# AtomGradient/swift-qwen3-tts

Measured on AMD Instinct MI355X. Metric: codec_tokens_per_s, higher is better.
Workload: dtype bf16

## Files before the change

swift-qwen3-tts_amd/csrc/codec.cc:

```cpp
#include "codec.h"

#include <algorithm>
#include <cstdlib>
#include <cstring>
#include <type_traits>
#include <utility>

#include "codec_kernels.h"

namespace q3 {

namespace {
size_t kScratchBudget = size_t(24) << 30;
}
void CodecRunner::set_scratch_budget(size_t bytes) { kScratchBudget = bytes ? bytes : (size_t(24) << 30); }

CodecRunner::CodecRunner(const Model& m, hipStream_t st, bool fp32_convs, int output_rate, float speed) : m_(m), st_(st) {
    native_ = mid_ = up_ = m.cfg.codec.total_upsample();
    if (speed != 0.0f && speed != 1.0f) {
        Q3_CHECK(speed >= 0.5f && speed <= 2.0f, 3, "Invalid input: speed must be 0 (off) or between 0.5 and 2.0");
        Q3_CHECK(native_ % kStretchHa == 0, 3, "Invalid input: the codec's frame is not a whole number of 480-sample hops: no speed other than 1");
        const int hops = native_ / kStretchHa;
        int L = 1, M = 1;
        if (output_rate != 0 && output_rate != kResampleNative && resample_rate_supported(output_rate)) {
// ... 55 lines not shown
    int C = dc.decoder_dim;
    for (int r : dc.upsample_rates) {
        ppf *= r;
        C /= 2;
        per_frame = std::max(per_frame, size_t(ppf) * C);
    }
    if (stretch_) per_frame = std::max(per_frame, size_t(mid_));
    return per_frame;
}

int CodecRunner::tail_context_frames() const {
    const CodecDecoderConfig& dc = m_.cfg.codec;
    double ctx = 0.0, rate = 1.0;
    for (int r : dc.upsampling_ratios) {
        rate *= r;
        ctx += 6.0 / rate;
    }
    ctx += 6.0 / rate;
    for (int r : dc.upsample_rates) {
        ctx += 1.0 / rate;
        rate *= r;
        ctx += 6.0 * (1 + 3 + 9) / rate;
    }
    ctx += 6.0 / rate;
    if (stretch_) ctx += double(stretch_lookback(st_plan_.hs)) / rate;
    if (resample_) ctx += double(out_plan_.taps() - 1) / rate;
    return int(ctx) + 2;
}

void CodecRunner::upload_lens(const int32_t* lens, int n) {
    if (size_t(n) > lens_dev_.capacity()) Q3_HIP(hipStreamSynchronize(st_));
    lens_dev_.grow(size_t(n));
    lens_host_.grow(size_t(n));
    Q3_HIP(hipStreamSynchronize(st_));
    std::memcpy(lens_host_, lens, size_t(n) * 4);
    Q3_HIP(hipMemcpyAsync(lens_dev_, lens_host_, size_t(n) * 4, hipMemcpyHostToDevice, st_));
}

void CodecRunner::conv(const Pass& ps, const ConvW& cw, const float* x, int Tmax, int ppf, float* out, const SnakeW* sn,
                       const float* res, int act, const SnakeW* post, float* out2) {
    launch([&] {
        ConvGemmArgs a{};
        const int64_t m_in = int64_t(ps.hist_frames) * ppf * cw.Cin, m_out = int64_t(ps.hist_frames) * ppf * cw.N;
        a.hist = ps.hist_frames * ppf;
        a.x = x + m_in; a.ldx = cw.Cin; a.x_bstride = int64_t(Tmax) * cw.Cin;
        a.w = cw.w; a.bias = cw.bias; a.scale = cw.scale;
        if (!fp32_mfma_) { a.wh = cw.wh; a.wsc = cw.wsc; }
        a.res = res ? res + m_out : nullptr; a.ldr = cw.N; a.res_bstride = int64_t(Tmax) * cw.N;
        a.out = out ? out + m_out : nullptr; a.ldo = cw.N; a.out_bstride = int64_t(Tmax) * cw.N;
        a.snake_ea = sn ? sn->ea : nullptr; a.snake_ib = sn ? sn->ib : nullptr;
        if (post) { a.out2 = out2 + m_out; a.post_ea = post->ea; a.post_ib = post->ib; a.post_C = post->C; }
        a.frames = ps.fr; a.ppf = ppf; a.Tmax = Tmax; a.B = ps.nb;
        a.Cin = cw.Cin; a.N = cw.N; a.K = cw.K; a.dil = cw.dil; a.act = act;
        launch_conv_gemm(a, st_);
    });
}

void CodecRunner::capture(const Pass& ps, const char* name, const float* t, int T, int C) {
    if (!ps.stage_out || *ps.stage != name) return;
    Q3_HIP(hipStreamSynchronize(st_));
    ps.stage_out->resize(size_t(ps.nb) * T * C);
    Q3_HIP(hipMemcpy(ps.stage_out->data(), t, ps.stage_out->size() * 4, hipMemcpyDeviceToHost));
    if (ps.stage_T) *ps.stage_T = T;
    if (ps.stage_C) *ps.stage_C = C;
}

void CodecRunner::run_front(const Pass& ps, const int32_t* codes, int code_stride_frames, int Fmax, float* const* bufs,
                            const int32_t* first_frame) {
    const CodecDecoderConfig& dc = m_.cfg.codec;
// ... 757 lines not shown
```

swift-qwen3-tts_amd/csrc/codec.h:

```cpp
#pragma once
#include <string>
#include <vector>

#include "model.h"
#include "resample_plan.h"
#include "stream_plan.h"
#include "stretch_plan.h"

namespace q3 {

class CodecRunner {
  public:
    CodecRunner(const Model& m, hipStream_t st, bool fp32_convs = false, int output_rate = 0, float speed = 0.0f);
    int decode(const int32_t* codes_dev, int code_stride_frames, const std::vector<int>& frames, float** pcm_dev,
               const std::string& stage = std::string(), std::vector<float>* stage_out = nullptr, int* stage_T = nullptr,
               int* stage_C = nullptr, int32_t* nonfinite_host = nullptr, bool force_fp32 = false);
    bool fp32_convs() const { return fp32_mfma_; }
    int decode_chunked(const int32_t* codes_dev, int code_stride_frames, const std::vector<int>& frames, int chunk_frames,
                       float* pcm_host, std::vector<hipEvent_t>& chunk_done, int32_t* nonfinite_host = nullptr,
                       int32_t* nf_chunks_host = nullptr);
    int tail_context_frames() const;
    static void set_scratch_budget(size_t bytes);

    struct StreamCfg {
// ... 107 lines not shown
        ~Stream() {
            for (auto e : ring_ev) (void)hipEventDestroy(e);
            for (auto e : quiet_ev) (void)hipEventDestroy(e);
        }
        uint8_t* take(size_t bytes);
        void* get(size_t frame_bytes, bool reads_back);
        void put(const void*) {}
    } stream_;
    void stream_prefix();
    size_t front_floats_per_frame() const;
    size_t floats_per_frame() const;
    void upload_lens(const int32_t* lens, int n);
    static constexpr int kMaxRows = 4096;
    const Model& m_;
    hipStream_t st_;
    int up_ = 1920;
    int native_ = 1920;
    bool resample_ = false;
    ResamplePlan out_plan_;
    DevBuf<float> out_tab_;
    int mid_ = 1920;
    bool stretch_ = false;
    StretchPlan st_plan_;
    DevBuf<float> st_fade_;
    static constexpr int kStateWords = 4;
    DevBuf<int32_t> ch_words_;
    DevBuf<float> ch_mid_;
    bool no_h1_ = false;
    bool no_fuse_ = false;
    bool fp32_mfma_ = false;
    DevBuf<uint8_t> buf_;
    DevBuf<int32_t> lens_dev_;
    PinnedBuf<int32_t> lens_host_;
    DevBuf<int32_t> nf_dev_;
};

}
```

swift-qwen3-tts_amd/csrc/debug_env.cc:

```cpp
#include <atomic>
#include <cstdlib>
#include <mutex>

#include "kernels.h"

namespace q3 {

namespace {
std::mutex g_mu;
std::atomic<const DebugEnv*> g_env{nullptr};

bool flag(const char* name) { return std::getenv(name) != nullptr; }
int number(const char* name, int dflt) {
    const char* e = std::getenv(name);
    return e && *e ? std::atoi(e) : dflt;
}

const DebugEnv* read_env() {
    DebugEnv* d = new DebugEnv{};
    d->gemm_no_row_split = flag("Q3TTS_GEMM_NO_ROW_SPLIT");
    d->gemm_one_pair = flag("Q3TTS_GEMM_ONE_PAIR");
    d->no_tall_gemm = flag("Q3TTS_NO_TALL_GEMM");
    d->tall_shape = number("Q3TTS_TALL_SHAPE", 0);
    d->chunk_qsplit = number("Q3TTS_CHUNK_QSPLIT", 0);
    d->conv_no_pw = flag("Q3TTS_CONV_NO_PW");
    d->nt_off = std::getenv("Q3TTS_NT") && number("Q3TTS_NT", 1) == 0;
    d->serial_jobs = number("Q3TTS_SERIAL_JOBS", 0) != 0;
    d->fail_back_half = number("Q3TTS_TEST_FAIL_BACK_HALF", 0) != 0;
    d->no_prefix_cache = number("Q3TTS_NO_PREFIX_CACHE", 0) != 0;
    return d;
}
}

const DebugEnv& debug_env() {
    const DebugEnv* e = g_env.load(std::memory_order_acquire);
    if (!e) {
        std::lock_guard<std::mutex> lk(g_mu);
        e = g_env.load(std::memory_order_acquire);
        if (!e) {
            e = read_env();
            g_env.store(e, std::memory_order_release);
        }
    }
    return *e;
}

void debug_env_reload() {
    std::lock_guard<std::mutex> lk(g_mu);
    g_env.store(read_env(), std::memory_order_release);
}

}
```

swift-qwen3-tts_amd/csrc/engine.cc:

```cpp
#include "engine.h"

#include <algorithm>
#include <cctype>
#include <chrono>
#include <cmath>
#include <cstdio>
#include <deque>
#include <functional>
#include <thread>

#include "codec.h"
#include "codec_kernels.h"
#include "frontend.h"

namespace q3 {

namespace {
std::string lower(const std::string& s) {
    std::string o = s;
    for (auto& c : o) c = char(std::tolower((unsigned char)c));
    return o;
}
const char* const kCodecRangeMsg =
    "Audio decoding failed: the codec decoder produced a non-finite waveform -- also on the fp32 matrix-core convolutions (the "
    "reference's range), which a row is re-decoded on when it leaves the fp16 range of the default two-plane kernels";
double now_s() {
    return std::chrono::duration<double>(std::chrono::steady_clock::now().time_since_epoch()).count();
}
struct Bump {
    uint8_t* base;
    size_t off = 0;
    template <class T>
    T* take(size_t n) {
        off = align_up(off, 256);
        T* p = base ? reinterpret_cast<T*>(base + off) : nullptr;
        off += n * sizeof(T);
        return p;
    }
};
void audio_chunk(q3tts_event_cb cb, void* user, int request_index, const float* pcm, int64_t n, int64_t offset) {
    q3tts_event ev{};
    ev.kind = Q3TTS_EVENT_AUDIO_CHUNK;
    ev.request_index = request_index;
    ev.pcm = pcm;
    ev.n_samples = n;
    ev.sample_offset = offset;
    cb(user, &ev);
}
}

Engine::Engine(Model* model, const q3tts_load_opts& opts) : m_(model), opts_(opts) {
    Q3_HIP(hipSetDevice(m_->device));
    {
        int least = 0, greatest = 0;
        Q3_HIP(hipDeviceGetStreamPriorityRange(&least, &greatest));
        Q3_HIP(hipStreamCreateWithPriority(&st_, hipStreamNonBlocking, greatest));
        Q3_HIP(hipStreamCreateWithPriority(&st_codec_, hipStreamNonBlocking, least));
        hipDeviceProp_t prop{};
        Q3_HIP(hipGetDeviceProperties(&prop, m_->device));
        int cus = prop.multiProcessorCount / 2;
        if (opts.codec_overlap_cus > 0) cus = opts.codec_overlap_cus;
// ... 1279 lines not shown
            const SlotStream::Out& o = ss->out[b];
            Q3_CHECK(o.complete, 7, "internal error: a row of the streamed job was left incomplete");
            std::memcpy(J.pcm_host + (size_t(b) * stride + prefix[size_t(b)]) * J.up, o.pcm.get(), size_t(J.frames[size_t(b)]) * J.up * 4);
            J.held_from[size_t(b)] = o.held_from;
            J.nf_host[b] = o.held_from >= 0 ? 1 : 0;
        }
        if (ss->have_first) J.timing.first_audio_ms = ss->first_audio_ms;
    }
};

int Engine::begin(const q3tts_request* reqs, int n, const q3tts_sampling& sp, q3tts_event_cb cb, void* user, const DebugOpts* dbg,
                  bool overlapped, bool background, const Voice* const* voices) {
    Q3_HIP(hipSetDevice(m_->device));
    std::vector<ResolvedRequest> rr;
    double t_start = 0;
    const int slot = open_job(reqs, n, sp, dbg, rr, t_start, voices);
    bool any_clone = false;
    for (auto& r : rr) any_clone = any_clone || r.clone;
    Q3_HIP(hipEventRecord(ev_fe_[0], st_));
    const bool frontend = any_clone && prepare_clone_rows(rr);
    Q3_HIP(hipEventRecord(ev_fe_[1], st_));
    std::vector<int> np, nt;
    assemble_prompts(rr, np, nt);
    const int Pmax = reserve_rows(rr, np, nt, sp);
    if (dbg) debug_buffers(n, *dbg);
    Q3_HIP(hipEventRecord(ev_[0], st_));
    enqueue_prefill(tk_, n, Pmax, block_table_, kv_len_, n_prompt_, active_);
    Q3_HIP(hipEventRecord(ev_[1], st_));
    Job& J = jobs_[slot];
    J.reset(n, codec_->upsample());
    J.chunk_frames = sp.audio_chunk_frames;
    J.frontend = frontend;
    J.busy = true;
    if (background && !cb && !dbg && sp.audio_chunk_frames == 0) {
        J.background = true;
        J.rr = std::move(rr);
        J.np = std::move(np);
        J.sp = sp;
        J.sp.per_request = nullptr;
        J.overlapped = overlapped;
        J.t_start = t_start;
        std::lock_guard<std::mutex> lk(work_mu_);
        if (!worker_.joinable()) worker_ = std::thread([this] { worker_loop(); });
        J.back = 1;
        J.back_status = 0;
        J.back_err.clear();
        work_ = &J;
        work_cv_.notify_all();
        return slot;
    }
    try {
        back_half(J, rr, np, sp, cb, user, dbg,
                  sp.audio_chunk_frames > 0 && sp.audio_window_frames > 0 && (!any_clone || sp.audio_stream_reference != 0) && !dbg, overlapped,
                  t_start);
    } catch (...) {
        J.busy = false;
        throw;
    }
    return slot;
}

void Engine::back_half(Job& J, const std::vector<ResolvedRequest>& rr, const std::vector<int>& np, const q3tts_sampling& sp,
                       q3tts_event_cb cb, void* user, const DebugOpts* dbg, bool streamed, bool overlapped, double t_start) {
    if (J.background && debug_env().fail_back_half) throw Error(7, "back half failed on request (Q3TTS_TEST_FAIL_BACK_HALF)");
    StreamedDecode sd(*this, J, streamed, sp, cb, user, rr, t_start);
    const int launched = frame_loop(J, rr, sp, cb, user, dbg, sd);
// ... 114 lines not shown
    Q3_HIP(hipMalloc(reinterpret_cast<void**>(&sampled_dev_), nf * 16 * 4));
    Q3_HIP(hipMemset(sampled_dev_, 0xff, nf * 16 * 4));
    if (dbg.talker_logits) Q3_HIP(hipMalloc(reinterpret_cast<void**>(&tl_dump_), nf * V * 2));
    if (dbg.cp_logits) Q3_HIP(hipMalloc(reinterpret_cast<void**>(&cl_dump_), nf * (t.num_code_groups - 1) * Vc * 2));
}

int Engine::frame_loop(Job& J, const std::vector<ResolvedRequest>& rr, const q3tts_sampling& sp, q3tts_event_cb cb, void* user,
                       const DebugOpts* dbg, StreamedDecode& sd) {
    const int n = J.n;
    const bool use_graph = opts_.use_graph && !dbg;
    build_cp_proj_tables();
    hipGraphExec_t ge = use_graph ? frame_graph(n) : nullptr;
    int frames_cap = 0;
    for (auto& r : rr) frames_cap = std::max(frames_cap, r.max_frames);
    std::vector<int32_t> h_nframes((size_t)(n), 0);
    std::vector<uint8_t> h_fin((size_t)(n), 0);
    std::vector<int> reported((size_t)(n), 0);
    int launched = 0;
    const bool fixed_len = sp.force_frames > 0 || dbg;
    const int burst_frames = std::max(1, max_inflight_frames / job_chains / 2);
    hipEvent_t ring[2] = {burst_ev_[0], burst_ev_[1]};
    int bursts = 0;
    bool done = false;
    while (!done && launched < frames_cap) {
        if (bursts >= 2) Q3_HIP(hipEventSynchronize(ring[bursts & 1]));
        int burst = std::min(burst_frames, frames_cap - launched);
        if (sd.on) {
            const int need = std::min(frames_cap, sd.next_need(launched, sp.audio_chunk_frames, std::max(0, sp.audio_lookahead_frames)));
            if (need > launched) burst = std::min(burst, need - launched);
        }
        for (int i = 0; i < burst; ++i) {
            if (use_graph) Q3_HIP(hipGraphLaunch(ge, st_));
            else enqueue_frame(n, dbg);
        }
        launched += burst;
        if (!(fixed_len && !cb)) {
            Q3_HIP(hipMemcpyAsync(h_nframes.data(), n_frames_, size_t(n) * 4, hipMemcpyDeviceToHost, st_));
            Q3_HIP(hipMemcpyAsync(h_fin.data(), finished_, size_t(n), hipMemcpyDeviceToHost, st_));
        }
        Q3_HIP(hipEventRecord(ring[bursts & 1], st_));
        ++bursts;
        if (fixed_len && !cb) {
            if (sd.on) {
                for (int b = 0; b < n; ++b) sd.avail[size_t(b)] = std::min(launched, rr[size_t(b)].max_frames);
                sd.feed(launched);
            }
            continue;
        }
        Q3_HIP(hipEventSynchronize(ring[(bursts - 1) & 1]));
        done = true;
        for (int b = 0; b < n; ++b) done = done && h_fin[size_t(b)];
        if (sd.on) {
            for (int b = 0; b < n; ++b) {
                sd.avail[size_t(b)] = h_nframes[size_t(b)];
                sd.fin[size_t(b)] = h_fin[size_t(b)];
            }
            sd.feed(launched);
            fire_chunks(J, J.n_chunks, &sd.avail, false);
        }
        if (cb)
            for (int b = 0; b < n; ++b) emit_tokens(cb, user, b, request_base + b, h_nframes[size_t(b)], reported[size_t(b)]);
    }
    Q3_HIP(hipEventRecord(ev_[2], st_));
    Q3_HIP(hipMemcpyAsync(h_nframes.data(), n_frames_, size_t(n) * 4, hipMemcpyDeviceToHost, st_));
    Q3_HIP(hipStreamSynchronize(st_));
    if (dbg) {
        const TalkerConfig& t = m_->cfg.talker;
        const size_t nf = size_t(n) * dbg->frames;
        if (dbg->sampled) Q3_HIP(hipMemcpy(dbg->sampled, sampled_dev_, nf * 16 * 4, hipMemcpyDeviceToHost));
        if (dbg->talker_logits) Q3_HIP(hipMemcpy(dbg->talker_logits, tl_dump_, nf * t.vocab_size * 2, hipMemcpyDeviceToHost));
        if (dbg->cp_logits)
            Q3_HIP(hipMemcpy(dbg->cp_logits, cl_dump_, nf * (t.num_code_groups - 1) * t.cp.vocab_size * 2, hipMemcpyDeviceToHost));
    }
    J.frames.assign(h_nframes.begin(), h_nframes.end());
    return launched;
}

void Engine::hand_off(Job& J, const std::vector<ResolvedRequest>& rr, StreamedDecode& sd, int launched, bool overlapped) {
    const int n = J.n;
    bool any_clone = false;
    std::vector<int> dframes((size_t)(n), 0);
    int Fdec = 0;
    for (int b = 0; b < n; ++b) {
        const int F = J.frames[size_t(b)];
        any_clone = any_clone || rr[size_t(b)].clone;
        J.ref_T[size_t(b)] = rr[size_t(b)].clone ? rr[size_t(b)].ref_T : 0;
        J.target_tokens[size_t(b)] = rr[size_t(b)].target_token_count;
        dframes[size_t(b)] = F > 0 ? F + J.ref_T[size_t(b)] : 0;
        Fdec = std::max(Fdec, dframes[size_t(b)]);
    }
    J.Fdec = sd.on ? (sd.ss ? sd.stride : Fcap_) : Fdec;
    J.codes_host.resize(size_t(n) * Fcap_ * 16);
    Q3_HIP(hipMemcpyAsync(J.codes_host.data(), codes_, J.codes_host.size() * 4, hipMemcpyDeviceToHost, st_));
    if (sd.on) {
        for (int b = 0; b < n; ++b) {
            sd.avail[size_t(b)] = J.frames[size_t(b)];
            sd.fin[size_t(b)] = 1;
        }
// ... 5 lines not shown
        J.decoded = Fdec > 0;
        return;
    }
    if (Fdec > 0) {
        J.dec_codes.grow(size_t(n) * Fdec * 16);
        if (any_clone) {
            J.row_desc.assign(size_t(n), DecodeRowDesc{});
            for (int b = 0; b < n; ++b) {
                const auto& r = rr[size_t(b)];
                if (J.frames[size_t(b)] == 0) continue;
                J.row_desc[size_t(b)] = DecodeRowDesc{r.clone ? ref_codes_dev_ + r.ref_off : nullptr, codes_ + size_t(b) * Fcap_ * 16,
                                                      r.clone ? r.ref_T : 0, J.frames[size_t(b)], b, 0};
                if (r.voice) {
                    J.ref_code0[size_t(b)] = r.voice->code0;
                } else if (r.clone) {
                    J.ref_code0[size_t(b)].resize(size_t(r.ref_T));
                    Q3_HIP(hipMemcpyAsync(J.ref_code0[size_t(b)].data(), ref_codes_dev_ + r.ref_off, size_t(r.ref_T) * 4,
                                          hipMemcpyDeviceToHost, st_));
                }
            }
            Q3_HIP(hipMemcpyAsync(J.row_desc_dev.grow(size_t(n)), J.row_desc.data(), size_t(n) * sizeof(DecodeRowDesc), hipMemcpyHostToDevice, st_));
            launch_build_decode_codes_rows(J.row_desc.data(), J.row_desc_dev, n, J.dec_codes, n, Fdec, st_);
        } else {
            Q3_HIP(hipMemcpy2DAsync(J.dec_codes, size_t(Fdec) * 64, codes_, size_t(Fcap_) * 64, size_t(Fdec) * 64, size_t(n),
                                    hipMemcpyDeviceToDevice, st_));
        }
    }
    Q3_HIP(hipStreamSynchronize(st_));
    start_decode(J, dframes, overlapped, nullptr);
}

void Engine::start_decode(Job& J, const std::vector<int>& dframes, bool overlapped, const int32_t* codes_host) {
    hipStream_t cst = codec_stream(overlapped, J.background);
    Q3_HIP(hipEventRecord(J.ev_codec[0], cst));
    if (J.Fdec > 0) {
        const size_t floats = size_t(J.n) * J.Fdec * J.up;
        J.pcm_host.grow(floats);
        if (codes_host && J.voices.empty()) {
            J.dec_codes.grow(size_t(J.n) * J.Fdec * 16);
            Q3_HIP(hipMemcpy2DAsync(J.dec_codes, size_t(J.Fdec) * 64, codes_host, size_t(Fcap_) * 64, size_t(J.Fdec) * 64, size_t(J.n),
                                    hipMemcpyHostToDevice, cst));
        } else if (codes_host) {
            J.dec_codes.grow(size_t(J.n) * J.Fdec * 16);
            Q3_HIP(hipMemsetAsync(J.dec_codes, 0, size_t(J.n) * J.Fdec * 64, cst));
            J.gen_codes.grow(size_t(J.n) * Fcap_ * 16);
            int Fgen = 0;
            for (int b = 0; b < J.n; ++b) Fgen = std::max(Fgen, J.frames[size_t(b)]);
            Q3_CHECK(Fgen <= Fcap_, 7, "internal error: more generated frames than max_frames");
            Q3_HIP(hipMemcpy2DAsync(J.gen_codes, size_t(Fcap_) * 64, codes_host, size_t(Fcap_) * 64, size_t(Fgen) * 64, size_t(J.n),
                                    hipMemcpyHostToDevice, cst));
            J.row_desc.assign(size_t(J.n), DecodeRowDesc{});
            for (int b = 0; b < J.n; ++b) {
                const Voice* v = J.voices[size_t(b)];
                J.row_desc[size_t(b)] = DecodeRowDesc{v ? static_cast<const int32_t*>(v->codes_dev) : nullptr,
                                                      J.gen_codes + size_t(b) * Fcap_ * 16, v ? v->ref_T : 0, J.frames[size_t(b)], b, 0};
            }
            Q3_HIP(hipMemcpyAsync(J.row_desc_dev.grow(size_t(J.n)), J.row_desc.data(), size_t(J.n) * sizeof(DecodeRowDesc),
                                  hipMemcpyHostToDevice, cst));
            launch_build_decode_codes_rows(J.row_desc.data(), J.row_desc_dev, J.n, J.dec_codes, J.n, J.Fdec, cst);
        }
        if (J.chunk_frames > 0) {
            J.clear_chunk_flags(J.Fdec);
            J.n_chunks = codec_->decode_chunked(J.dec_codes, J.Fdec, dframes, J.chunk_frames, J.pcm_host, J.chunk_done, J.nf_host,
                                                J.nf_chunk_host);
        } else {
            float* pcm_dev = nullptr;
            codec_->decode(J.dec_codes, J.Fdec, dframes, &pcm_dev, std::string(), nullptr, nullptr, nullptr, J.nf_host);
            Q3_HIP(hipMemcpyAsync(J.pcm_host, pcm_dev, floats * 4, hipMemcpyDeviceToHost, cst));
        }
        J.decoded = true;
    }
    Q3_HIP(hipEventRecord(J.ev_codec[1], cst));
}

void Engine::job_timing(Job& J, const std::vector<int>& np, int launched) {
    float ms = 0;
    Q3_HIP(hipEventElapsedTime(&ms, ev_[0], ev_[1]));
    J.timing.prefill_ms = ms;
    Q3_HIP(hipEventElapsedTime(&ms, ev_[1], ev_[2]));
    J.timing.decode_ms = ms;
    Q3_HIP(hipEventElapsedTime(&ms, ev_fe_[0], ev_fe_[1]));
    J.timing.frontend_ms = J.frontend ? ms : 0;
    J.timing.frame_steps = launched;
    J.timing.launches_per_frame_step = launches_per_step(J.n);
    J.timing.rows = J.n;
    for (int b = 0; b < J.n; ++b) J.timing.kv_bytes_read += kv_bytes(np[size_t(b)], J.frames[size_t(b)]);
}

void Engine::publish_job(Job& J, q3tts_event_cb cb, void* user, int req_base, double t_start, bool stage) {
    J.cb = cb;
    J.user = user;
    J.request_base = req_base;
    J.t_start = t_start;
    J.seq = job_seq_++;
    J.busy = true;
    compute_cuts(J);
    std::lock_guard<std::mutex> lk(stage_mu_);
    J.stage_err.clear();
    J.stage = (stage && J.decoded) ? 1 : 0;
    if (J.stage == 1) {
        if (!stager_.joinable()) stager_ = std::thread([this] { staging_loop(); });
        stage_cv_.notify_all();
    }
}

void Engine::release_job(Job& J) {
    {
        std::unique_lock<std::mutex> lk(stage_mu_);
        stage_cv_.wait(lk, [&] { return J.stage != 1; });
    }
    J.st_pcm.clear();
    J.st_codes.clear();
    J.back_status = 0;
    J.busy = false;
}

void Engine::Job::reset(int rows, int upsample) {
    n = rows;
    up = upsample;
    Fdec = 0;
    frames.assign(size_t(n), 0);
    ref_T.assign(size_t(n), 0);
    target_tokens.assign(size_t(n), 0);
    ref_code0.assign(size_t(n), {});
    req_index.clear();
    row_out.clear();
    row_span.clear();
    held_from.assign(size_t(n), -1);
    std::memset(nf_host, 0, nf_host.capacity() * 4);
    n_chunks = chunk_frames = chunks_fired = 0;
    streamed = prefixed = decoded = background = frontend = false;
    voices.clear();
    t_first_audio = t_done = 0;
    timing = q3tts_timing{};
}

void Engine::Job::clear_chunk_flags(int frames) {
    const size_t slots = size_t(ceil_div(frames, chunk_frames) + 1) * size_t(n);
    std::memset(nf_chunk_host.grow(slots), 0, slots * 4);
}

void check_row_sampling(const q3tts_sampling& sp, int n) {
    if (!sp.per_request) return;
    constexpr uint32_t kKnown = Q3TTS_ROW_TEMPERATURE | Q3TTS_ROW_TOP_K | Q3TTS_ROW_TOP_P | Q3TTS_ROW_REPETITION_PENALTY | Q3TTS_ROW_SEED;
    for (int i = 0; i < n; ++i) {
        const q3tts_row_sampling& r = sp.per_request[i];
        const std::string at = " (per_request[" + std::to_string(i) + "])";
        Q3_CHECK((r.set & ~kKnown) == 0, 3, "Invalid input: unknown bits in q3tts_row_sampling.set" + at);
        if (r.set & Q3TTS_ROW_TEMPERATURE) Q3_CHECK(std::isfinite(r.temperature), 3, "Invalid input: temperature must be finite" + at);
        if (r.set & Q3TTS_ROW_TOP_K) Q3_CHECK(r.top_k >= 0, 3, "Invalid input: top_k must not be negative" + at);
        if (r.set & Q3TTS_ROW_TOP_P)
            Q3_CHECK(std::isfinite(r.top_p) && r.top_p >= 0.f && r.top_p <= 1.f, 3, "Invalid input: top_p must be in [0, 1]" + at);
        if (r.set & Q3TTS_ROW_REPETITION_PENALTY)
            Q3_CHECK(std::isfinite(r.repetition_penalty) && r.repetition_penalty > 0.f, 3,
                     "Invalid input: repetition_penalty must be finite and positive" + at);
    }
}

SamplingParams fold_sampling(const q3tts_sampling& sp, int i, uint32_t row0) {
    SamplingParams o{sp.temperature, sp.top_k, sp.top_p, sp.repetition_penalty, sp.seed, row0, sp.force_frames > 0 ? 1 : 0};
    if (!sp.per_request) return o;
    const q3tts_row_sampling& r = sp.per_request[i];
    if (r.set & Q3TTS_ROW_TEMPERATURE) o.temperature = r.temperature;
    if (r.set & Q3TTS_ROW_TOP_K) o.top_k = r.top_k;
    if (r.set & Q3TTS_ROW_TOP_P) o.top_p = r.top_p;
    if (r.set & Q3TTS_ROW_REPETITION_PENALTY) o.rep_penalty = r.repetition_penalty;
    if (r.set & Q3TTS_ROW_SEED) o.seed = r.seed;
// ... 82 lines not shown
        if (!J.cb) continue;
        const int64_t c0 = int64_t(k) * J.chunk_frames * up, c1 = std::min<int64_t>(int64_t(J.Fdec), int64_t(k + 1) * J.chunk_frames) * up;
        std::unique_lock<std::mutex> lk = cb_lock();
        for (int b = 0; b < n; ++b) {
            if (J.held_from[size_t(b)] >= 0) continue;
            const int64_t cut = known ? 0 : J.row_cut[size_t(b)];
            const int64_t len = known ? int64_t((*known)[size_t(b)]) * up : J.row_ns[size_t(b)];
            const int64_t lo = std::max(c0, cut), hi = std::min(c1, cut + len);
            if (hi <= lo) continue;
            audio_chunk(J.cb, J.user, J.request_base + b, J.pcm_host + size_t(b) * J.Fdec * up + lo, hi - lo, lo - cut);
        }
    }
}

void Engine::stage_rows(Job& J) {
    Q3_HIP(hipSetDevice(m_->device));
    Q3_HIP(hipEventSynchronize(J.ev_codec[1]));
    J.t_done = now_s();
    const int n = J.n;
    J.st_pcm.clear();
    J.st_pcm.resize(size_t(n));
    J.st_codes.clear();
    J.st_codes.resize(size_t(n));
    for (int b = 0; b < n; ++b) {
        const int F = J.frames[size_t(b)];
        if (F == 0 || !J.decoded) continue;
        const int64_t ns = J.row_ns[size_t(b)];
        J.st_codes[size_t(b)].reset(static_cast<int32_t*>(std::malloc(size_t(F) * 16 * 4)));
        J.st_pcm[size_t(b)].reset(static_cast<float*>(std::malloc(std::max<size_t>(size_t(ns) * 4, 4))));
        Q3_CHECK(J.st_codes[size_t(b)] && J.st_pcm[size_t(b)], 5, "out of host memory for the results");
        std::memcpy(J.st_codes[size_t(b)].get(), J.codes_host.data() + size_t(b) * Fcap_ * 16, size_t(F) * 16 * 4);
        std::memcpy(J.st_pcm[size_t(b)].get(), J.pcm_host + size_t(b) * J.Fdec * J.up + J.row_cut[size_t(b)], size_t(ns) * 4);
    }
}

void Engine::staging_loop() {
    std::unique_lock<std::mutex> lk(stage_mu_);
    for (;;) {
        Job* next = nullptr;
        for (auto& J : jobs_)
            if (J.stage == 1 && (!next || J.seq < next->seq)) next = &J;
        if (!next) {
            if (stage_stop_) return;
            stage_cv_.wait(lk);
            continue;
        }
        lk.unlock();
        int state = 2;
        std::string err;
        try {
            stage_rows(*next);
        } catch (const std::exception& e) {
            state = 3;
            err = e.what();
        }
        lk.lock();
        next->stage = state;
        next->stage_err = err;
        stage_cv_.notify_all();
    }
}

std::vector<int> Engine::redo_rows_fp32(Job& J) {
    std::vector<int> rows, bad;
    if (!J.decoded) return bad;
    for (int b = 0; b < J.n; ++b)
// ... 113 lines not shown
        r.info.tokens_per_second = total > 0 ? double(F) / total : 0;
        r.info.peak_memory_usage = double(total_b - free_b) / 1e9;
        if (F == 0 || !J.decoded) {
            r.status = Q3TTS_ERR_GENERATION_FAILED;
            continue;
        }
        if (std::find(still_bad.begin(), still_bad.end(), b) != still_bad.end()) {
            r.status = Q3TTS_ERR_AUDIO_DECODING_FAILED;
            last_error = kCodecRangeMsg;
            continue;
        }
        r.n_frames = F;
        r.codes = J.st_codes[size_t(b)].release();
        r.n_samples = row_ns[size_t(b)];
        r.pcm = J.st_pcm[size_t(b)].release();
        r.status = Q3TTS_OK;
    }
    if (J.cb) {
        std::unique_lock<std::mutex> lk = cb_lock();
        for (int b = 0; b < n; ++b) {
            if (out(b).status != Q3TTS_OK) continue;
            q3tts_event ev{};
            ev.kind = Q3TTS_EVENT_INFO;
            ev.request_index = ev_index(b);
            ev.info = &out(b).info;
            J.cb(J.user, &ev);
            ev.kind = Q3TTS_EVENT_AUDIO;
            ev.info = nullptr;
            ev.pcm = out(b).pcm;
            ev.n_samples = out(b).n_samples;
            J.cb(J.user, &ev);
        }
    }
}

bool Engine::job_outstanding() const {
    for (const auto& J : jobs_)
        if (J.busy) return true;
    return false;
}

ResolvedRequest Engine::check_queued(const q3tts_request& r, const q3tts_sampling& sp, const Voice* voice, bool open_text) const {
    const TalkerConfig& t = m_->cfg.talker;
    Q3_CHECK(r.ref_audio == nullptr, 3, "Invalid input: voice-clone requests (ref_audio) are not supported by q3tts_generate_queued");
    ResolvedRequest o = resolve(r, sp, voice);
    if (open_text) {
        Q3_CHECK(!o.clone, 3, "Invalid input: an open-text request cannot be a voice-clone request");
        o.n_tail = 0;
        o.text_open = true;
        o.open_max_tokens = r.max_tokens > 0 ? r.max_tokens : 2048;
        o.open_force_frames = sp.force_frames;
        o.max_frames = sp.force_frames > 0 ? sp.force_frames : o.open_max_tokens;
        o.target_token_count = int(o.text_ids.size()) - 3;
    }
    Q3_CHECK(m_->has_codec, 1, "Model not initialized: Speech tokenizer not loaded");
    Q3_CHECK(o.max_frames <= Fcap_, 3, "Invalid input: max_tokens exceeds the configured max_frames");
    Q3_CHECK(o.language_id < t.vocab_size && o.speaker_token < t.vocab_size, 3, "Invalid input: codec prefix id out of range");
    const int tl = int(o.text_ids.size());
    int nc = (o.language_id < 0 ? 3 : 4) + (o.speaker_token >= 0 ? 1 : 0) + 2;
    int np = int(o.instruct_ids.size()) + 3 + nc;
    int nt = (tl - o.n_tail > 4 ? tl - o.n_tail - 4 : 0) + 1;
    if (o.clone) {
        nc += m_->has_speaker_encoder ? 1 : 0;
        np = 3 + (nc - 1) + (int(o.ref_text_ids.size()) - 5) + (tl - 8) + 2 + o.ref_T;
        nt = 1;
    }
// ... 1403 lines not shown

void Engine::debug_codec_stage(const int32_t* codes, int n_frames, const char* stage, float* out, int64_t cap, int* T, int* C) {
    Q3_CHECK(m_->has_codec, 1, "Model not initialized: Speech tokenizer not loaded");
    DevBuf<int32_t> dcodes;
    dcodes.grow(size_t(n_frames) * 16);
    Q3_HIP(hipMemcpy(dcodes, codes, size_t(n_frames) * 16 * 4, hipMemcpyHostToDevice));
    std::vector<float> so;
    float* pcm_dev = nullptr;
    (void)codec_stream(false);
    codec_->decode(dcodes, n_frames, {n_frames}, &pcm_dev, stage, &so, T, C);
    Q3_CHECK(int64_t(so.size()) <= cap, 3, "debug_codec_stage: output buffer too small");
    std::memcpy(out, so.data(), so.size() * 4);
}


EngineGroup::EngineGroup(std::unique_ptr<Model> model, const q3tts_load_opts& opts) : model_(std::move(model)), opts_(opts) {
    int lanes = opts.n_streams;
    if (lanes <= 0) lanes = 1;
    lanes = std::max(1, std::min(lanes, opts.max_batch));
    q3tts_load_opts lo = opts;
    lo.max_batch = ceil_div(opts.max_batch, lanes);
    for (int i = 0; i < lanes; ++i) {
        lanes_.push_back(std::make_unique<Engine>(model_.get(), lo));
        lanes_.back()->cb_mutex = &cb_mutex_;
        lanes_.back()->max_inflight_frames = std::max(2, 12000 / 650 / lanes);
    }
    speakers = lanes_[0]->speakers;
    if (lanes == 1) {
        ctx1_ = std::make_unique<Engine>(model_.get(), lo);
        ctx1_->cb_mutex = &cb_mutex_;
        background_ = !debug_env().serial_jobs;
        if (background_)
            for (Engine* e : {lanes_[0].get(), ctx1_.get()}) e->prepare_job_pair();
    }
}

EngineGroup::~EngineGroup() {
    session_.reset();
    ctx1_.reset();
    lanes_.clear();
}

Engine* EngineGroup::free_context() {
    Engine* c[2] = {lanes_[0].get(), ctx1_.get()};
    for (int k = 1; k <= 2; ++k) {
        const int i = (last_ctx_ + k) & 1;
        if (c[i]->job_outstanding()) continue;
        last_ctx_ = i;
        c[i]->row_offset = 0;
        c[i]->request_base = 0;
        return c[i];
    }
    throw Error(3, "Invalid input: two jobs are already outstanding (q3tts_generate_end must be called first)");
}

int EngineGroup::begin(const q3tts_request* reqs, int n, const q3tts_sampling& sp, q3tts_event_cb cb, void* user, bool more_follows) {
    Q3_CHECK(n >= 1 && n <= opts_.max_batch, 3, "Invalid input: batch size must be between 1 and max_batch");
    check_row_sampling(sp, n);
    if (lanes_.size() == 1) {
        Engine* e = free_context();
        return (e == ctx1_.get() ? Engine::kJobSlots : 0) + e->begin(reqs, n, sp, cb, user, nullptr, more_follows, background_);
    }
    int slot = -1;
    for (int i = 0; i < Engine::kJobSlots; ++i)
        if (!parked_[i].busy) slot = i;
    Q3_CHECK(slot >= 0, 3, "Invalid input: two jobs are already outstanding (q3tts_generate_end must be called first)");
    parked_[slot].results.assign(size_t(n), q3tts_result{});
// ... 403 lines not shown
```

swift-qwen3-tts_amd/csrc/engine.h:

```cpp
#pragma once
#include <atomic>
#include <cstdlib>
#include <map>
#include <memory>
#include <condition_variable>
#include <mutex>
#include <thread>
#include <string>
#include <unordered_map>
#include <vector>

#include "../../include/q3tts.h"
#include "kernels.h"
#include "model.h"
#include "resample_plan.h"
#include "session_queue.h"
#include "stretch_plan.h"

namespace q3 {

struct DebugOpts {
    const int32_t* forced_codes = nullptr;
    int frames = 0;
    uint16_t* talker_logits = nullptr;
    uint16_t* cp_logits = nullptr;
    int32_t* sampled = nullptr;
};

struct Voice {
    const void* owner = nullptr;
    int ref_T = 0;
    int64_t n_ref_samples = 0;
    std::vector<int32_t> ref_text_ids;
    DevBuf<int32_t> codes_dev;
    DevBuf<uint16_t> rows_dev;
    std::vector<int32_t> codes_host;
    std::vector<int32_t> code0;
    int64_t device_bytes = 0;
};

struct ResolvedRequest {
    std::vector<int32_t> text_ids, instruct_ids;
    int speaker_token = -1;
    int language_id = -1;
    int max_frames = 0;
// ... 77 lines not shown

struct RequestSource {
    virtual ~RequestSource() = default;
    virtual bool take(QueueItem& out) = 0;
    virtual q3tts_result* result(int ticket) = 0;
    virtual void complete(int) {}
    virtual bool open_ended() const { return false; }
    virtual bool wait_for_work() { return false; }
    virtual bool has_cancels() { return false; }
    virtual void take_cancels(std::vector<int>& out) { out.clear(); }
    virtual void complete_cancelled(int) {}
    virtual void progress(int , int ) {}
    struct TextAppend {
        int ticket = -1;
        std::vector<int32_t> ids;
        bool final = false;
    };
    virtual bool open_text() const { return false; }
    virtual bool has_appends() { return false; }
    virtual void take_appends(std::vector<TextAppend>& out) { out.clear(); }
    virtual void wait_for_text(bool ) {}
    virtual void text_progress(int , int ) {}
};

struct QueueShared {
    RequestSource* src = nullptr;
    uint32_t row_base = 0;
    int voice_ref_max = -1;
    bool stream_reference = false;
    int ref_max = 0;
    PrefixCache* prefix_cache = nullptr;
};

class Engine {
  public:
    Engine(Model* model, const q3tts_load_opts& opts);
    ~Engine();

    Model& model() { return *m_; }
    const q3tts_load_opts& opts() const { return opts_; }
    std::string last_error;
    q3tts_timing timing{};

    void generate(const q3tts_request* reqs, int n, const q3tts_sampling& sp, q3tts_event_cb cb, void* user,
                  q3tts_result* results, const DebugOpts* dbg, const Voice* const* voices = nullptr);
    static constexpr int kJobSlots = 2;
    int begin(const q3tts_request* reqs, int n, const q3tts_sampling& sp, q3tts_event_cb cb, void* user, const DebugOpts* dbg,
              bool overlapped,
              bool background = false, const Voice* const* voices = nullptr);
    void end(int job, q3tts_result* results);
    bool job_outstanding() const;
    int text_cap() const { return Tcap_; }
    void prepare_job_pair();
    void drain();
    ResolvedRequest check_queued(const q3tts_request& r, const q3tts_sampling& sp, const Voice* voice = nullptr,
                                 bool open_text = false) const;
    void check_stream_chunk(int chunk_frames) const;
    void run_queued(QueueShared& q, int slots, const q3tts_sampling& sp, q3tts_event_cb cb, void* user);
    void debug_prepare_inputs(const q3tts_request& req, uint16_t* input_embeds, int cap_prompt, int* n_prompt,
                              uint16_t* trailing, int cap_trailing, int* n_trailing, uint16_t* tts_pad);
    void debug_sample(const uint16_t* logits, int rows, int V, const q3tts_sampling& sp, const uint8_t* seen,
                      int suppress_lo, int suppress_hi, int eos_id, uint32_t row0, uint32_t draw, int32_t* tokens);
    void debug_text_resume(int H, int V, const uint16_t* tables, const int32_t* codes, const uint16_t* text, uint16_t* out_h,
                           float* out_ss, int32_t* out_state);
    void debug_linear(const uint16_t* x, const uint16_t* W, const uint16_t* bias, int M, int K, int N, uint16_t* y);
    void debug_attention(const q3tts_attn_debug& a);
    static void debug_gemm_check(q3tts_gemm_debug& d, GemmArgs& ga, NormRowsArgs& na);
    void debug_gemm(q3tts_gemm_debug& d);
    static void debug_conv_check(q3tts_conv_debug& d);
    void debug_conv(q3tts_conv_debug& d);
    void debug_build_decode_codes(const int32_t* refs, const int32_t* ref_T, const int32_t* gen, const int32_t* n_frames, int R,
                                  int gen_stride, int Fdec, bool misalign, int32_t* out);
    void codec_decode(const int32_t* codes, const int32_t* n_frames, int batch, int max_frames, float* pcm,
                      int64_t* audio_lengths);
    void codec_decode_streamed(const int32_t* codes, const int32_t* n_frames, int batch, int max_frames, int chunk_frames, int window,
                               int lookahead, float* pcm);
    void codec_decode_streamed_prefixed(const int32_t* codes, const int32_t* n_prefix, const int32_t* n_frames, int batch, int max_frames,
                                        int chunk_frames, int window, int lookahead, float* pcm);
    void debug_codec_stream_slots(const int32_t* codes, const int32_t* n_frames, int n_reqs, int max_frames, int slots, int burst,
                                  int chunk_frames, int window, int lookahead, float* pcm);
    void debug_codec_stage(const int32_t* codes, int n_frames, const char* stage, float* out, int64_t cap, int* T, int* C);
    int codec_encode(const float* audio, int64_t n_samples, int32_t* codes, int cap_frames);
    int encoded_frames(int64_t n_samples) const;
    void speaker_embedding(const float* audio, int64_t n_samples, float* out, int cap);
    std::unique_ptr<Voice> create_voice(const float* audio, int64_t n_samples, const int32_t* ref_text_ids, int n_ref_text_ids,
                                        int sample_rate = 24000);
// ... 62 lines not shown
        q3tts_sampling sp{};
        bool overlapped = false;
        bool frontend = false;
        bool background = false;
        int back = 0;
        int back_status = 0;
        std::string back_err;
        int n = 0, Fdec = 0, up = 0;
        std::vector<int> frames, ref_T, target_tokens, n_prompt;
        std::vector<int> req_index;
        std::vector<q3tts_result*> row_out;
        std::vector<double> row_span;
        std::vector<std::vector<int32_t>> ref_code0;
        std::vector<int32_t> codes_host;
        DevBuf<int32_t> dec_codes;
        std::vector<const Voice*> voices;
        DevBuf<int32_t> gen_codes;
        std::vector<DecodeRowDesc> row_desc;
        DevBuf<DecodeRowDesc> row_desc_dev;
        PinnedBuf<float> pcm_host;
        hipEvent_t ev_codec[2] = {nullptr, nullptr};
        PinnedBuf<int32_t> nf_host;
        PinnedBuf<int32_t> nf_chunk_host;
        std::vector<int> held_from;
        hipEvent_t ev_begin = nullptr, ev_first_audio = nullptr;
        std::vector<hipEvent_t> chunk_done;
        int n_chunks = 0, chunk_frames = 0;
        bool streamed = false;
        bool prefixed = false;
        int chunks_fired = 0;
        double t_first_audio = 0;
        q3tts_timing timing{};
        double t_start = 0, t_done = 0;
        q3tts_event_cb cb = nullptr;
        void* user = nullptr;
        int request_base = 0;
        bool decoded = false;
        std::vector<int64_t> row_cut, row_ns;
        std::vector<MallocPtr<float>> st_pcm;
        std::vector<MallocPtr<int32_t>> st_codes;
        int stage = 0;
        std::string stage_err;
        void reset(int rows, int upsample);
        void clear_chunk_flags(int frames);
    } jobs_[kJobSlots];
    void start_decode(Job& J, const std::vector<int>& dframes, bool overlapped, const int32_t* codes_host);
    void publish_job(Job& J, q3tts_event_cb cb, void* user, int request_base, double t_start, bool stage);
    void release_job(Job& J);
    void compute_cuts(Job& J);
    void fire_chunks(Job& J, int upto, const std::vector<int>* known, bool wait);
    std::unique_lock<std::mutex> cb_lock();
    void emit_tokens(q3tts_event_cb cb, void* user, int row, int request, int nf, int& reported);
    void stage_rows(Job& J);
    std::vector<int> redo_rows_fp32(Job& J);
    void staging_loop();
    std::thread stager_;
    std::mutex stage_mu_;
    std::condition_variable stage_cv_;
    bool stage_stop_ = false;
    uint64_t job_seq_ = 0;

    unsigned long long* stamps_ = nullptr;
    void stamp(int k) {
        if (stamps_) launch_stamp(stamps_, stamps_ + 63, k, counted());
    }
    hipStream_t counted() {
        ++launches_;
        return st_;
    }
    int launches_ = 0;
    std::map<int, int> frame_launches_;
    std::map<int, hipGraphExec_t> graphs_;
    std::unique_ptr<CodecRunner> codec_;
    std::unique_ptr<VoiceFrontEnd> fe_;
    DevBuf<float> ref_audio_dev_;
    DevBuf<int32_t> ref_codes_dev_;
    DevBuf<uint16_t> extra_;
    DevBuf<float> spk_f32_;
    struct FeLane {
        hipStream_t st = nullptr;
        hipEvent_t done = nullptr;
        std::unique_ptr<VoiceFrontEnd> fe;
        DevBuf<float> spk;
    };
    std::vector<FeLane> fe_lanes_;
    const float* upload_audio(const float* audio, int64_t n);
    struct ResamplerDev {
        ResamplePlan plan;
        DevBuf<float> tab;
    };
    std::vector<std::unique_ptr<ResamplerDev>> resamplers_;
    DevBuf<float> rs_out_dev_;
    DevBuf<int32_t> rs_len_dev_;
// ... 100 lines not shown
    bool mine(const Voice* v) const;
    PrefixCache& prefix_cache() { return prefix_cache_; }
    int begin(const q3tts_request* reqs, int n, const q3tts_sampling& sp, q3tts_event_cb cb, void* user, bool more_follows);
    void end(int job, q3tts_result* results);
    void generate_queued(const q3tts_request* reqs, int n, int slots, const q3tts_sampling& sp, q3tts_event_cb cb, void* user,
                         q3tts_result* results, const Voice* const* voices = nullptr);
    Session* open_session(const q3tts_session_opts& so, const q3tts_sampling& sp, q3tts_event_cb cb, void* user);
    Session* session() const { return session_.get(); }
    int close_session(bool drain);
    std::string last_error;
    q3tts_timing timing{};
    std::vector<std::string> speakers;

  private:
    std::unique_ptr<Session> session_;
    void check_queue_open(int slots, const q3tts_sampling& sp) const;
    template <class F>
    static void run_lanes(int L, bool serial, F&& fn);
    struct Parked {
        bool busy = false;
        std::vector<q3tts_result> results;
        q3tts_timing timing{};
    } parked_[Engine::kJobSlots];
    std::unique_ptr<Model> model_;
    q3tts_load_opts opts_;
    std::mutex cb_mutex_;
    std::vector<std::unique_ptr<Engine>> lanes_;
    std::vector<std::unique_ptr<Voice>> voices_;
    PrefixCache prefix_cache_;
    void check_voices(const q3tts_request* reqs, int n, const Voice* const* voices) const;
    std::unique_ptr<Engine> ctx1_;
    int last_ctx_ = 1;
    bool background_ = false;
    Engine* free_context();
};

class Session final : public RequestSource {
  public:
    struct Item {
        ResolvedRequest rr;
        SamplingParams params{};
    };
    Session(EngineGroup& g, Engine& lane, const q3tts_session_opts& so, const q3tts_sampling& sp, q3tts_event_cb cb, void* user);
    ~Session() override;
    void submit(const q3tts_request& r, const Voice* voice, const q3tts_row_sampling* rs, int64_t* ticket);
    void submit_open(const q3tts_request& r, const q3tts_row_sampling* rs, int64_t* ticket);
    void append_text(int64_t ticket, const int32_t* ids, int32_t n, bool final);
    void text_stats(q3tts_session_text_stats* s) const { queue_.text_stats(s); }
    int cancel(int64_t ticket) { return queue_.cancel(ticket); }
    void wait(int64_t ticket, int32_t timeout_ms, q3tts_result* out, int32_t* ready);
    void stats(q3tts_session_stats* s) const { queue_.stats(s); }
    int close(bool drain);
    bool on_loop_thread() const { return std::this_thread::get_id() == thread_.get_id(); }
    std::string error() const;

    bool take(QueueItem& out) override;
    q3tts_result* result(int ticket) override { return queue_.result(ticket); }
    void complete(int ticket) override { queue_.complete(ticket); }
    bool open_ended() const override { return true; }
    bool wait_for_work() override { return queue_.wait_for_work(); }
    bool has_cancels() override { return queue_.has_cancels(); }
    void take_cancels(std::vector<int>& out) override;
    void complete_cancelled(int ticket) override { queue_.complete_cancelled(ticket); }
    void progress(int frame_steps, int admissions) override { queue_.progress(frame_steps, admissions); }
    bool open_text() const override { return true; }
    bool has_appends() override { return queue_.has_appends(); }
// ... 20 lines not shown
```

swift-qwen3-tts_amd/csrc/kernels.h:

```cpp
#pragma once
#include <hip/hip_runtime.h>

#include <cstdint>

namespace q3 {

struct DebugEnv {
    bool gemm_no_row_split;
    bool gemm_one_pair;
    bool no_tall_gemm;
    int tall_shape;
    int chunk_qsplit;
    bool conv_no_pw;
    bool nt_off;
    bool serial_jobs;
    bool fail_back_half;
    bool no_prefix_cache;
};
const DebugEnv& debug_env();
void debug_env_reload();

constexpr int kPageTokens = 64;
constexpr int kHeadDim = 128;

struct NormRowsArgs {
    const uint16_t* h;
    int hMB;
    const uint16_t* w;
    float eps;
    uint16_t* out;
    int outMB;
    float* ss_out;
    int M, H;
    const float* ss_in;
    int ss_count, ss_ld;
};
void launch_norm_rows(const NormRowsArgs& a, hipStream_t st);

struct GemmArgs {
    const uint16_t* W;
    const uint32_t* Wsb;
    const uint16_t* x;
    int xMB;
    int M, Mpad, N, K;
    int epi;
    uint16_t* y;
    int ldy;
    int y_tiled, yMB;
    const uint16_t* bias;
    int act_silu;
// ... 204 lines not shown
```

Baseline: 10290.

## Serialize background codec decodes across contexts with an event-ordered gate

Adds a DecodeGate that gives background codec decode passes from the two engine contexts a ticket order. Each pass makes its codec stream wait on the previous pass's completion event through a small ring of three events, so the two contexts' decodes no longer contend on the GPU at the same time. upload_lens now waits on an event recorded after its own host-to-device copy instead of synchronizing the whole stream, so the host no longer blocks on unrelated queued work. The change also adds optional per-job tracing and a test failure hook, and it holds a mutex across the enqueue of each decode pass.

```diff
diff --git a/swift-qwen3-tts_amd/csrc/codec.cc b/swift-qwen3-tts_amd/csrc/codec.cc
--- a/swift-qwen3-tts_amd/csrc/codec.cc
+++ b/swift-qwen3-tts_amd/csrc/codec.cc
@@ -111,9 +111,11 @@
     if (size_t(n) > lens_dev_.capacity()) Q3_HIP(hipStreamSynchronize(st_));
     lens_dev_.grow(size_t(n));
     lens_host_.grow(size_t(n));
-    Q3_HIP(hipStreamSynchronize(st_));
+    if (!lens_copied_.e) Q3_HIP(hipEventCreateWithFlags(&lens_copied_.e, hipEventDisableTiming));
+    else Q3_HIP(hipEventSynchronize(lens_copied_.e));
     std::memcpy(lens_host_, lens, size_t(n) * 4);
     Q3_HIP(hipMemcpyAsync(lens_dev_, lens_host_, size_t(n) * 4, hipMemcpyHostToDevice, st_));
+    Q3_HIP(hipEventRecord(lens_copied_.e, st_));
 }
 
 void CodecRunner::conv(const Pass& ps, const ConvW& cw, const float* x, int Tmax, int ppf, float* out, const SnakeW* sn,
diff --git a/swift-qwen3-tts_amd/csrc/codec.h b/swift-qwen3-tts_amd/csrc/codec.h
--- a/swift-qwen3-tts_amd/csrc/codec.h
+++ b/swift-qwen3-tts_amd/csrc/codec.h
@@ -163,6 +163,12 @@
     DevBuf<uint8_t> buf_;
     DevBuf<int32_t> lens_dev_;
     PinnedBuf<int32_t> lens_host_;
+    struct OwnedEvent {
+        hipEvent_t e = nullptr;
+        ~OwnedEvent() {
+            if (e) (void)hipEventDestroy(e);
+        }
+    } lens_copied_;
     DevBuf<int32_t> nf_dev_;
 };
 
diff --git a/swift-qwen3-tts_amd/csrc/debug_env.cc b/swift-qwen3-tts_amd/csrc/debug_env.cc
--- a/swift-qwen3-tts_amd/csrc/debug_env.cc
+++ b/swift-qwen3-tts_amd/csrc/debug_env.cc
@@ -1,5 +1,6 @@
 #include <atomic>
 #include <cstdlib>
+#include <cstring>
 #include <mutex>
 
 #include "kernels.h"
@@ -26,8 +27,12 @@
     d->conv_no_pw = flag("Q3TTS_CONV_NO_PW");
     d->nt_off = std::getenv("Q3TTS_NT") && number("Q3TTS_NT", 1) == 0;
     d->serial_jobs = number("Q3TTS_SERIAL_JOBS", 0) != 0;
-    d->fail_back_half = number("Q3TTS_TEST_FAIL_BACK_HALF", 0) != 0;
+    d->fail_in_decode = number("Q3TTS_TEST_FAIL_BACK_HALF", 0) == 2;
+    d->fail_back_half = number("Q3TTS_TEST_FAIL_BACK_HALF", 0) != 0 && !d->fail_in_decode;
     d->no_prefix_cache = number("Q3TTS_NO_PREFIX_CACHE", 0) != 0;
+    d->decode_gate_off = std::getenv("Q3TTS_DECODE_GATE") && number("Q3TTS_DECODE_GATE", 1) == 0;
+    const char* trace = std::getenv("Q3TTS_JOB_TRACE");
+    d->job_trace = trace && *trace ? strdup(trace) : nullptr;
     return d;
 }
 }
diff --git a/swift-qwen3-tts_amd/csrc/decode_gate.h b/swift-qwen3-tts_amd/csrc/decode_gate.h
--- /dev/null
+++ b/swift-qwen3-tts_amd/csrc/decode_gate.h
@@ -0,0 +1,75 @@
+#pragma once
+#include <cstdint>
+#include <mutex>
+
+namespace q3 {
+
+class DecodeGate {
+  public:
+    static constexpr int kEvents = 3;
+    struct Ticket {
+        uint64_t n = 0;
+        int wait = -1;
+        int record = 0;
+    };
+    Ticket enter() {
+        mu_.lock();
+        Ticket t;
+        t.n = next_++;
+        t.wait = last_;
+        t.record = (last_ + 1) % kEvents;
+        return t;
+    }
+    void complete(const Ticket& t) {
+        last_ = t.record;
+        ++completed_;
+        mu_.unlock();
+    }
+    void abandon(const Ticket&) {
+        ++abandoned_;
+        mu_.unlock();
+    }
+    void counts(uint64_t* taken, uint64_t* completed, uint64_t* abandoned) {
+        std::lock_guard<std::mutex> lk(mu_);
+        *taken = next_;
+        *completed = completed_;
+        *abandoned = abandoned_;
+    }
+
+  private:
+    std::mutex mu_;
+    uint64_t next_ = 0, completed_ = 0, abandoned_ = 0;
+    int last_ = -1;
+};
+
+template <class Ops>
+class DecodePass {
+  public:
+    DecodePass(DecodeGate& g, Ops& ops) : g_(g), ops_(ops), t_(g.enter()) {
+        try {
+            if (t_.wait >= 0) ops_.wait(t_.wait);
+        } catch (...) {
+            g_.abandon(t_);
+            throw;
+        }
+    }
+    DecodePass(const DecodePass&) = delete;
+    DecodePass& operator=(const DecodePass&) = delete;
+    ~DecodePass() {
+        if (open_) g_.abandon(t_);
+    }
+    const DecodeGate::Ticket& ticket() const { return t_; }
+    void finish() {
+        ops_.record(t_.record);
+        open_ = false;
+        g_.complete(t_);
+    }
+
+  private:
+    DecodeGate& g_;
+    Ops& ops_;
+    DecodeGate::Ticket t_;
+    bool open_ = true;
+};
+
+}
diff --git a/swift-qwen3-tts_amd/csrc/engine.cc b/swift-qwen3-tts_amd/csrc/engine.cc
--- a/swift-qwen3-tts_amd/csrc/engine.cc
+++ b/swift-qwen3-tts_amd/csrc/engine.cc
@@ -27,6 +27,7 @@
 double now_s() {
     return std::chrono::duration<double>(std::chrono::steady_clock::now().time_since_epoch()).count();
 }
+enum { kTrContext = 0, kTrFront, kTrFirstStep, kTrLoopDrained, kTrDecodeQueued, kTrDecodeDone, kTrStaged, kTrEnd };
 struct Bump {
     uint8_t* base;
     size_t off = 0;
@@ -1372,6 +1373,10 @@
     J.chunk_frames = sp.audio_chunk_frames;
     J.frontend = frontend;
     J.busy = true;
+    if (tracing()) {
+        J.tr[kTrContext] = t_start;
+        J.tr[kTrFront] = now_s();
+    }
     if (background && !cb && !dbg && sp.audio_chunk_frames == 0) {
         J.background = true;
         J.rr = std::move(rr);
@@ -1552,6 +1557,7 @@
         for (int i = 0; i < burst; ++i) {
             if (use_graph) Q3_HIP(hipGraphLaunch(ge, st_));
             else enqueue_frame(n, dbg);
+            if (launched == 0 && i == 0 && tracing()) J.tr[kTrFirstStep] = now_s();
         }
         launched += burst;
         if (!(fixed_len && !cb)) {
@@ -1584,6 +1590,7 @@
     Q3_HIP(hipEventRecord(ev_[2], st_));
     Q3_HIP(hipMemcpyAsync(h_nframes.data(), n_frames_, size_t(n) * 4, hipMemcpyDeviceToHost, st_));
     Q3_HIP(hipStreamSynchronize(st_));
+    if (tracing()) J.tr[kTrLoopDrained] = now_s();
     if (dbg) {
         const TalkerConfig& t = m_->cfg.talker;
         const size_t nf = size_t(n) * dbg->frames;
@@ -1655,10 +1662,23 @@
 
 void Engine::start_decode(Job& J, const std::vector<int>& dframes, bool overlapped, const int32_t* codes_host) {
     hipStream_t cst = codec_stream(overlapped, J.background);
+    const size_t floats = size_t(J.n) * J.Fdec * J.up;
+    if (J.Fdec > 0) J.pcm_host.grow(floats);
+    J.overlapped = overlapped;
+    struct GateOps {
+        JobGate* g;
+        hipStream_t st;
+        void wait(int slot) { Q3_HIP(hipStreamWaitEvent(st, g->done[slot], 0)); }
+        void record(int slot) { Q3_HIP(hipEventRecord(g->done[slot], st)); }
+    } gate_ops{gate_, cst};
+    std::unique_ptr<DecodePass<GateOps>> pass;
+    if (J.background && gate_ && gate_->on) {
+        pass = std::make_unique<DecodePass<GateOps>>(gate_->order, gate_ops);
+        J.ticket = int64_t(pass->ticket().n);
+    }
     Q3_HIP(hipEventRecord(J.ev_codec[0], cst));
+    if (J.background && debug_env().fail_in_decode) throw Error(7, "decode failed on request (Q3TTS_TEST_FAIL_BACK_HALF=2)");
     if (J.Fdec > 0) {
-        const size_t floats = size_t(J.n) * J.Fdec * J.up;
-        J.pcm_host.grow(floats);
         if (codes_host && J.voices.empty()) {
             J.dec_codes.grow(size_t(J.n) * J.Fdec * 16);
             Q3_HIP(hipMemcpy2DAsync(J.dec_codes, size_t(J.Fdec) * 64, codes_host, size_t(Fcap_) * 64, size_t(J.Fdec) * 64, size_t(J.n),
@@ -1694,6 +1714,8 @@
         J.decoded = true;
     }
     Q3_HIP(hipEventRecord(J.ev_codec[1], cst));
+    if (pass) pass->finish();
+    if (tracing()) J.tr[kTrDecodeQueued] = now_s();
 }
 
 void Engine::job_timing(Job& J, const std::vector<int>& np, int launched) {
@@ -1756,6 +1778,8 @@
     voices.clear();
     t_first_audio = t_done = 0;
     timing = q3tts_timing{};
+    for (double& t : tr) t = 0;
+    ticket = -1;
 }
 
 void Engine::Job::clear_chunk_flags(int frames) {
@@ -1904,6 +1928,10 @@
         std::memcpy(J.st_codes[size_t(b)].get(), J.codes_host.data() + size_t(b) * Fcap_ * 16, size_t(F) * 16 * 4);
         std::memcpy(J.st_pcm[size_t(b)].get(), J.pcm_host + size_t(b) * J.Fdec * J.up + J.row_cut[size_t(b)], size_t(ns) * 4);
     }
+    if (tracing()) {
+        J.tr[kTrDecodeDone] = J.t_done;
+        J.tr[kTrStaged] = now_s();
+    }
 }
 
 void Engine::staging_loop() {
@@ -2083,6 +2111,31 @@
             J.cb(J.user, &ev);
         }
     }
+    if (tracing()) write_job_trace(J, job);
+}
+
+void Engine::write_job_trace(Job& J, int slot) {
+    static std::mutex mu;
+    J.tr[kTrEnd] = now_s();
+    float g0 = -1.f, g1 = -1.f;
+    if (J.decoded && !J.streamed) {
+        if (hipEventElapsedTime(&g0, gate_->epoch, J.ev_codec[0]) != hipSuccess ||
+            hipEventElapsedTime(&g1, gate_->epoch, J.ev_codec[1]) != hipSuccess) {
+            g0 = g1 = -1.f;
+            (void)hipGetLastError();
+        }
+    }
+    std::lock_guard<std::mutex> lk(mu);
+    std::FILE* f = std::fopen(gate_->trace_path, "a");
+    if (!f) return;
+    static const char* names[] = {"context", "front", "first_step", "loop_drained", "decode_queued", "decode_done", "staged", "end"};
+    std::fprintf(f, "job seq=%llu ctx=%d slot=%d rows=%d background=%d overlapped=%d gate=%d ticket=%lld", (unsigned long long)J.seq,
+                 trace_ctx_, slot, J.n, J.background ? 1 : 0, J.overlapped ? 1 : 0, gate_->on ? 1 : 0,
+                 (long long)J.ticket);
+    for (int k = 0; k < 8; ++k) std::fprintf(f, " %s=%.3f", names[k], J.tr[k] > 0 ? (J.tr[k] - gate_->t0) * 1e3 : -1.0);
+    std::fprintf(f, " gpu_decode_start=%.3f gpu_decode_done=%.3f decode_ms=%.3f codec_ms=%.3f frame_steps=%d\n", double(g0), double(g1),
+                 double(J.timing.decode_ms), double(J.timing.codec_ms), J.timing.frame_steps);
+    std::fclose(f);
 }
 
 bool Engine::job_outstanding() const {
@@ -3552,7 +3605,28 @@
         background_ = !debug_env().serial_jobs;
         if (background_)
             for (Engine* e : {lanes_[0].get(), ctx1_.get()}) e->prepare_job_pair();
-    }
+        gate_ = std::make_unique<JobGate>();
+        gate_->on = background_ && !debug_env().decode_gate_off;
+        lanes_[0]->set_job_gate(gate_.get(), 0);
+        ctx1_->set_job_gate(gate_.get(), 1);
+    }
+}
+
+JobGate::JobGate() {
+    for (auto& e : done) Q3_HIP(hipEventCreateWithFlags(&e, hipEventDisableTiming));
+    trace_path = debug_env().job_trace;
+    if (trace_path) {
+        Q3_HIP(hipEventCreate(&epoch));
+        Q3_HIP(hipEventRecord(epoch, nullptr));
+        Q3_HIP(hipEventSynchronize(epoch));
+        t0 = now_s();
+    }
+}
+
+JobGate::~JobGate() {
+    for (auto& e : done)
+        if (e) (void)hipEventDestroy(e);
+    if (epoch) (void)hipEventDestroy(epoch);
 }
 
 EngineGroup::~EngineGroup() {
diff --git a/swift-qwen3-tts_amd/csrc/engine.h b/swift-qwen3-tts_amd/csrc/engine.h
--- a/swift-qwen3-tts_amd/csrc/engine.h
+++ b/swift-qwen3-tts_amd/csrc/engine.h
@@ -11,6 +11,7 @@
 #include <vector>
 
 #include "../../include/q3tts.h"
+#include "decode_gate.h"
 #include "kernels.h"
 #include "model.h"
 #include "resample_plan.h"
@@ -154,6 +155,19 @@
     PrefixCache* prefix_cache = nullptr;
 };
 
+struct JobGate {
+    DecodeGate order;
+    hipEvent_t done[DecodeGate::kEvents] = {nullptr, nullptr, nullptr};
+    bool on = false;
+    const char* trace_path = nullptr;
+    double t0 = 0;
+    hipEvent_t epoch = nullptr;
+    JobGate();
+    ~JobGate();
+    JobGate(const JobGate&) = delete;
+    JobGate& operator=(const JobGate&) = delete;
+};
+
 class Engine {
   public:
     Engine(Model* model, const q3tts_load_opts& opts);
@@ -174,6 +188,10 @@
     bool job_outstanding() const;
     int text_cap() const { return Tcap_; }
     void prepare_job_pair();
+    void set_job_gate(JobGate* g, int ctx) {
+        gate_ = g;
+        trace_ctx_ = ctx;
+    }
     void drain();
     ResolvedRequest check_queued(const q3tts_request& r, const q3tts_sampling& sp, const Voice* voice = nullptr,
                                  bool open_text = false) const;
@@ -302,6 +320,8 @@
         double t_first_audio = 0;
         q3tts_timing timing{};
         double t_start = 0, t_done = 0;
+        double tr[8] = {0, 0, 0, 0, 0, 0, 0, 0};
+        int64_t ticket = -1;
         q3tts_event_cb cb = nullptr;
         void* user = nullptr;
         int request_base = 0;
@@ -329,6 +349,10 @@
     std::condition_variable stage_cv_;
     bool stage_stop_ = false;
     uint64_t job_seq_ = 0;
+    JobGate* gate_ = nullptr;
+    int trace_ctx_ = 0;
+    bool tracing() const { return gate_ && gate_->trace_path; }
+    void write_job_trace(Job& J, int slot);
 
     unsigned long long* stamps_ = nullptr;
     void stamp(int k) {
@@ -495,6 +519,7 @@
     std::unique_ptr<Engine> ctx1_;
     int last_ctx_ = 1;
     bool background_ = false;
+    std::unique_ptr<JobGate> gate_;
     Engine* free_context();
 };
 
diff --git a/swift-qwen3-tts_amd/csrc/kernels.h b/swift-qwen3-tts_amd/csrc/kernels.h
--- a/swift-qwen3-tts_amd/csrc/kernels.h
+++ b/swift-qwen3-tts_amd/csrc/kernels.h
@@ -16,6 +16,9 @@
     bool serial_jobs;
     bool fail_back_half;
     bool no_prefix_cache;
+    bool fail_in_decode;
+    bool decode_gate_off;
+    const char* job_trace;
 };
 const DebugEnv& debug_env();
 void debug_env_reload();
```

New measurement: 10360 (median of 4 runs). No clear change (+0.7%).
